# roboterax/humanoid-gym

Measured on AMD Instinct MI355X. Metric: env-steps/s (XBot-L PPO, whole job), higher is better.
Workload: dtype bf16

## Files before the change

humanoid-gym_amd/csrc/hgym_net.hip:

```cpp
#include <stdlib.h>

#include "hgym_gemm.hpp"
#include "hgym_fused.hpp"
#include "hgym_norm.hpp"
#include "hgym_loss.hpp"

namespace hgym {

int32_t launch_mlp_fb(const FwdArgs& fb, const FbLoss& fl, bool shadow, bool unclipped, int tiles, int nets, size_t lds, hipStream_t s);
int32_t launch_mlp_fb_act(const FwdArgs& fb, const FbLoss& fl, bool shadow, bool unclipped, int tiles, int nets, hipStream_t s, int first);
int32_t launch_ppo_loss_mirror(const LossArgs& a, bool bf16, bool unclipped, int nblocks, hipStream_t s);
int32_t launch_mlp_fwd_act(const FwdArgs& a, int nets, bool wide, int64_t dbg_tiles, hipStream_t s);
int32_t launch_bc_loss(const BcLossArgs& a, bool bf16, int nblocks, hipStream_t s);
int32_t launch_bc_scalars(const BcScalArgs& a, hipStream_t s);
int32_t launch_ppo_loss_smooth(const LossArgs& a, const LossSmooth& sm, bool bf16, int nblocks, hipStream_t s);
int32_t launch_perturb_rows(int64_t M, int width, const float* src, int64_t ld_src, const int64_t* idx, const float* noise_std, uint64_t seed,
                            const double* opt_state, float* dst, int64_t ld_dst, hipStream_t s);
int32_t launch_smooth_sums(int nblocks, int B, int A, const float* partials, const float* weight, double* sums, hipStream_t s);

struct LayerLayout {
    int K, N;
    int Kp, Ncp, N16, K16;
    int64_t w_off, b_off;
    int64_t Wp, WTp;
// ... 153 lines not shown
            if (n.fused) {
                y.KBf = l == 0 ? l0_ksteps(y.K).KB : (int)round_up(y.K, 32) / 32;
                y.KRf = l == 0 ? l0_ksteps(y.K).KR : y.KBf;
                y.NBf = y.N16 / 16;
                y.NBBf = (int)round_up(y.N, 32) / 32;
                y.Wf = take((int64_t)y.NBf * y.KBf * 1024);
                y.WTf = take((int64_t)y.K16 / 16 * y.NBBf * 1024);
            } else {
                y.Wp = take((int64_t)y.N16 * y.Kp * w->es);
                y.WTp = take((int64_t)y.K16 * y.Ncp * w->es);
                y.X = take(w->maxM * y.Kp * w->es);
                y.XT = take((int64_t)y.K16 * w->Mp * w->es);
                y.dY = take(w->maxM * y.Ncp * w->es);
                y.dYT = take((int64_t)y.N16 * w->Mp * w->es);
            }
        }
        n.out_f32 = take(w->maxM * (int64_t)dims[n.L] * 4);
        if (n.fused) {
            n.X0b = take(w->Mpad * (int64_t)n.layer[0].KBf * 32 * 2);
            for (int l = 0; l < 3; ++l) {
                n.Hb[l] = take(w->Mpad * (int64_t)n.layer[l].N * 2);
                n.dZb[l] = take(w->Mpad * (int64_t)n.layer[l].N * 2);
            }
            n.dZb[3] = take(w->Mpad * 32 * n.layer[3].NBBf * 2);
        }
    }
    w->P = poff;
    if (w->aux_p0 < 0) w->aux_p0 = poff;
    w->Ps = round_up(poff, 64);
    w->splits = MAX_SPLITS;
    w->dw_splits = 8;
    w->slabs = take((int64_t)w->splits * w->Ps * 4);
    w->partials = take((int64_t)MAX_LOSS_BLOCKS * LOSS_PARTIALS * 4);
    w->zeros = take(4096);
    w->sqn = take((SQN_BLOCKS + 2) * 8);
    w->sigma = c->std_param == HGYM_STD_LOG ? take(SIGMA_FLOATS * 4) : -1;
    w->total_bytes = off;
    return HGYM_OK;
}

__global__ __launch_bounds__(1024) void fin_only_kernel(const FinArgs f) { fin_block(f, threadIdx.x, blockDim.x); }

template <typename T>
__global__ __launch_bounds__(256) void pack_rows_kernel(int M, int K, const float* __restrict__ src, int64_t ld_src,
                                                        const int64_t* __restrict__ idx, T* __restrict__ dst, int64_t ld_dst) {
    const int64_t total = (int64_t)M * K;
    for (int64_t i = (int64_t)blockIdx.x * blockDim.x + threadIdx.x; i < total; i += (int64_t)gridDim.x * blockDim.x) {
        const int m = (int)(i / K), k = (int)(i - (int64_t)m * K);
        const int64_t r = idx ? idx[m] : m;
        dst[(int64_t)m * ld_dst + k] = from_f32<T>(src[r * ld_src + k]);
    }
}

template <typename T>
__global__ __launch_bounds__(256) void transpose_kernel(int M, int Mp, int C, const T* __restrict__ in, int64_t ld_in,
                                                        T* __restrict__ out, int64_t ld_out) {
    __shared__ T tile[64][66];
    const int m0 = blockIdx.x * 64, c0 = blockIdx.y * 64;
    const int tx = threadIdx.x & 63, ty = threadIdx.x >> 6;
    for (int r = ty; r < 64; r += 4) {
        const int m = m0 + r, c = c0 + tx;
        tile[r][tx] = (m < M && c < C) ? in[(int64_t)m * ld_in + c] : from_f32<T>(0.0f);
    }
    __syncthreads();
    for (int r = ty; r < 64; r += 4) {
        const int c = c0 + r, m = m0 + tx;
        if (c < C && m < Mp) out[(int64_t)c * ld_out + m] = tile[tx][r];
    }
}

template <typename T>
__global__ __launch_bounds__(256) void rowsum_kernel(int Mp, int per, const T* __restrict__ in, int64_t ld_in, float* __restrict__ out,
                                                     int64_t slab_stride) {
    constexpr int V = 16 / sizeof(T);
    __shared__ float red[4];
    const T* row = in + (int64_t)blockIdx.y * ld_in;
    float s = 0.0f;
    for (int c = 0; c < per; ++c) {
        const int base = (blockIdx.x * per + c) * (256 * 4 * V);
#pragma unroll
        for (int u = 0; u < 4; ++u) {
            const int m = base + (u * 256 + threadIdx.x) * V;
            if (m < Mp) {
                const u32x4 raw = *reinterpret_cast<const u32x4*>(row + m);
                const T* e = reinterpret_cast<const T*>(&raw);
#pragma unroll
                for (int k = 0; k < V; ++k) s += to_f32<T>(e[k]);
            }
        }
    }
#pragma unroll
    for (int off = 32; off > 0; off >>= 1) s += __shfl_down(s, off, 64);
    if ((threadIdx.x & 63) == 0) red[threadIdx.x >> 6] = s;
    __syncthreads();
    if (threadIdx.x == 0) out[(int64_t)blockIdx.x * slab_stride + blockIdx.y] = red[0] + red[1] + red[2] + red[3];
}

template <typename T>
__global__ __launch_bounds__(256) void aux_mse_kernel(int B, int Bp, int No, const float* __restrict__ y, const float* __restrict__ priv,
                                                      int64_t ldp, int off, const int64_t* __restrict__ idx, float coef,
                                                      T* __restrict__ dY, int64_t ld, T* __restrict__ dYT, int64_t ldt,
                                                      double* __restrict__ opt) {
    __shared__ float red[4];
    const int i = blockIdx.x * blockDim.x + threadIdx.x;
    float se = 0.0f;
    if (i < B) {
        const float* t = priv + idx[i] * ldp + off;
        const float g = 2.0f * coef / ((float)B * (float)No);
        for (int j = 0; j < No; ++j) {
            const float d = y[(int64_t)i * No + j] - t[j];
            se += d * d;
            const T gv = from_f32<T>(g * d);
            dY[(int64_t)i * ld + j] = gv;
            dYT[(int64_t)j * ldt + i] = gv;
        }
    } else if (i < Bp) {
        for (int j = 0; j < No; ++j) dYT[(int64_t)j * ldt + i] = from_f32<T>(0.0f);
    }
#pragma unroll
    for (int o = 32; o > 0; o >>= 1) se += __shfl_down(se, o, 64);
    if ((threadIdx.x & 63) == 0) red[threadIdx.x >> 6] = se;
    __syncthreads();
    if (threadIdx.x == 0) atomicAdd(&opt[HGYM_OPT_AUX_SUM], (double)(red[0] + red[1] + red[2] + red[3]) / ((double)B * (double)No));
}

__global__ __launch_bounds__(256) void act_sample_kernel(int M, int A, const float* __restrict__ mu, const float* __restrict__ std_,
                                                         const float* __restrict__ z, uint64_t seed, const int64_t* __restrict__ step,
                                                         float* __restrict__ actions, float* __restrict__ sigma, float* __restrict__ logp) {
    const int m = blockIdx.x * blockDim.x + threadIdx.x;
    if (m >= M) return;
    RngKey rk = {(uint32_t)seed, (uint32_t)(seed >> 32), 0u, 0u};
    if (!z) {
        const int64_t s = step ? step[0] : 0;
        rk.s0 = (uint32_t)s;
        rk.s1 = (uint32_t)(s >> 32);
    }
    float lp = 0.0f;
    float zn[16];
    if (!z) normals_block<4>(rk, (uint32_t)m, SLOT_POLICY, zn);
#pragma unroll
    for (int j = 0; j < 16; ++j) {
        if (j >= A) break;
        const float mj = mu[(int64_t)m * A + j];
        const float sg = mj * 0.0f + std_[j];
        const float zz = z ? z[(int64_t)m * A + j] : zn[j];
        const float a = mj + sg * zz;
        actions[(int64_t)m * A + j] = a;
        sigma[(int64_t)m * A + j] = sg;
        const float d = a - mj;
        lp += -(d * d) / (2.0f * sg * sg) - logf(sg) - 0.9189385332046727f;
    }
    logp[m] = lp;
}


__global__ __launch_bounds__(512) void ppo_scalars_kernel(const ScalArgs a) { ppo_scalars_block(a, threadIdx.x, blockDim.x); }

struct Segment {
    int64_t off;
    int rows, cols;
    int splits;
    void* Wp;
    int64_t ldw;
    void* WTp;
    int64_t ldwt;
    void* Wf;
    void* WTf;
    int KB, NBB;
    float* sigma;
};
struct SegTable {
    int n;
    Segment s[2 * HGYM_MAX_LAYERS * 2 + 1];
};
struct NormCols {
    const float* cs[2 * HGYM_MAX_LAYERS * 2 + 1];
};

__global__ __launch_bounds__(256) void reduce_slabs_kernel(const SegTable tab, int64_t P, const float* __restrict__ slabs,
                                                           float* __restrict__ grads, double* __restrict__ opt) {
    __shared__ double red[4];
    const Segment& sg = tab.s[blockIdx.y];
    const int64_t n = (int64_t)sg.rows * sg.cols;
    const int64_t stride = (int64_t)gridDim.x * blockDim.x;
    double sq = 0.0;
    if (sg.splits == 0) {
        for (int64_t i = (int64_t)blockIdx.x * blockDim.x + threadIdx.x; i < n; i += stride) {
            const float g = grads[sg.off + i];
            sq += (double)g * (double)g;
        }
    } else {
        const bool vec = (P & 3) == 0 && (((uintptr_t)grads | (uintptr_t)slabs) & 15) == 0;
        const int64_t head = vec ? ((4 - (sg.off & 3)) & 3) < n ? ((4 - (sg.off & 3)) & 3) : n : n;
        const int64_t n4 = (n - head) >> 2, tail0 = head + 4 * n4;
        const int64_t base = sg.off + head;
        for (int64_t i = (int64_t)blockIdx.x * blockDim.x + threadIdx.x; i < n4; i += stride) {
            float4 acc = make_float4(0.f, 0.f, 0.f, 0.f);
            if (sg.splits == 8) {
                float4 v[8];
#pragma unroll
                for (int z = 0; z < 8; ++z) v[z] = *reinterpret_cast<const float4*>(slabs + (int64_t)z * P + base + 4 * i);
#pragma unroll
                for (int z = 0; z < 8; ++z) { acc.x += v[z].x; acc.y += v[z].y; acc.z += v[z].z; acc.w += v[z].w; }
            } else {
                for (int z = 0; z < sg.splits; ++z) {
                    const float4 v = *reinterpret_cast<const float4*>(slabs + (int64_t)z * P + base + 4 * i);
                    acc.x += v.x; acc.y += v.y; acc.z += v.z; acc.w += v.w;
                }
            }
            *reinterpret_cast<float4*>(grads + base + 4 * i) = acc;
            sq += (double)acc.x * (double)acc.x + (double)acc.y * (double)acc.y + (double)acc.z * (double)acc.z + (double)acc.w * (double)acc.w;
        }
        for (int64_t i = (int64_t)blockIdx.x * blockDim.x + threadIdx.x; i < head + (n - tail0); i += stride) {
            const int64_t e = i < head ? i : tail0 + (i - head);
            float s = 0.0f;
            for (int z = 0; z < sg.splits; ++z) s += slabs[(int64_t)z * P + sg.off + e];
            grads[sg.off + e] = s;
            sq += (double)s * (double)s;
        }
    }
#pragma unroll
    for (int off = 32; off > 0; off >>= 1) sq += __shfl_down(sq, off, 64);
    if ((threadIdx.x & 63) == 0) red[threadIdx.x >> 6] = sq;
    __syncthreads();
    if (threadIdx.x == 0) {
        double t = red[0] + red[1] + red[2] + red[3];
        t = __builtin_rint(t * 0x1p46) * 0x1p-46;
        if (t != 0.0) atomicAdd(&opt[HGYM_OPT_GRAD_SQNORM], t);
    }
}


__device__ __forceinline__ void apply_prologue(const HgymPPOConfig& p, const float* __restrict__ kl_slot, float inv_w, double* __restrict__ opt,
                                               int have_sq, double sq) {
    if (p.world_size > 1) opt[HGYM_OPT_KL_LAST] = (double)(kl_slot[0] * inv_w);
    if (PROLOGUE_PENDING(opt)) {
        if (have_sq >= 0) opt[HGYM_OPT_GRAD_SQNORM] = have_sq ? sq : 0.0;
        return;
    }
    if (p.adaptive_lr) opt[HGYM_OPT_LR] = adapt_lr(opt[HGYM_OPT_LR], (float)opt[HGYM_OPT_KL_LAST], p.desired_kl, p.lr_min, p.lr_max);
    const double t = opt[HGYM_OPT_STEP] + 1.0;
    opt[HGYM_OPT_STEP] = t;
    const bool cached = opt[HGYM_OPT_PROLOGUE_STEP] == t;
    const double bc1 = 1.0 - (cached ? opt[HGYM_OPT_BETA1_POW] : pow((double)p.beta1, t)), bc2 = 1.0 - (cached ? opt[HGYM_OPT_BETA2_POW] : pow((double)p.beta2, t));
    opt[HGYM_OPT_STEP_SIZE] = (double)(float)(opt[HGYM_OPT_LR] / bc1);
    opt[HGYM_OPT_SQRT_BC2] = (double)(float)sqrt(bc2);
    opt[HGYM_OPT_PROLOGUE_STEP] = t;
    if (have_sq >= 0) opt[HGYM_OPT_GRAD_SQNORM] = have_sq ? sq : 0.0;
}
__global__ void apply_prologue_kernel(const HgymPPOConfig p, const float* __restrict__ kl_slot, float inv_w, double* __restrict__ opt) {
    if (threadIdx.x != 0 || blockIdx.x != 0) return;
    apply_prologue(p, kl_slot, inv_w, opt, (p.world_size > 1 || !p.grad_norm_ready) ? 0 : -1, 0.0);
}

__global__ __launch_bounds__(256) void sqnorm_prologue_kernel(int64_t P, const float* __restrict__ g, float inv_w, const HgymPPOConfig p,
                                                              const float* __restrict__ kl_slot, double* __restrict__ opt,
                                                              double* __restrict__ part) {
    __shared__ double red[4];
    __shared__ unsigned int s_last;
    double s = 0.0;
    for (int64_t i = (int64_t)blockIdx.x * blockDim.x + threadIdx.x; i < P; i += (int64_t)gridDim.x * blockDim.x) {
        const float gi = g[i] * inv_w;
        s += (double)gi * (double)gi;
    }
#pragma unroll
    for (int off = 32; off > 0; off >>= 1) s += __shfl_down(s, off, 64);
    if ((threadIdx.x & 63) == 0) red[threadIdx.x >> 6] = s;
    __syncthreads();
    unsigned int* counter = reinterpret_cast<unsigned int*>(part + SQN_BLOCKS);
    if (threadIdx.x == 0) {
        part[blockIdx.x] = red[0] + red[1] + red[2] + red[3];
        __threadfence();
        s_last = atomicAdd(counter, 1u) == gridDim.x - 1u ? 1u : 0u;
    }
    __syncthreads();
    if (!s_last) return;
    __threadfence();
    double v = threadIdx.x < gridDim.x ? reinterpret_cast<const volatile double*>(part)[threadIdx.x] : 0.0;
#pragma unroll
    for (int off = 32; off > 0; off >>= 1) v += __shfl_down(v, off, 64);
    __syncthreads();
    if ((threadIdx.x & 63) == 0) red[threadIdx.x >> 6] = v;
    __syncthreads();
    if (threadIdx.x == 0) {
        *counter = 0u;
        apply_prologue(p, kl_slot, inv_w, opt, 1, red[0] + red[1] + red[2] + red[3]);
    }
}

__device__ __forceinline__ float sigma_of(float log_sigma) { return expf(log_sigma); }

template <typename T>
__device__ __forceinline__ void write_shadows(const Segment& sg, int r, int c, float w) {
    if (sg.Wp) {
        ((T*)sg.Wp)[(int64_t)r * sg.ldw + c] = from_f32<T>(w);
        if (sg.WTp) ((T*)sg.WTp)[(int64_t)c * sg.ldwt + r] = from_f32<T>(w);
    }
    if (sg.Wf) {
        ((T*)sg.Wf)[((((int64_t)(r >> 4) * sg.KB + (c >> 5)) * 64) + ((c & 31) >> 3) * 16 + (r & 15)) * 8 + (c & 7)] = from_f32<T>(w);
        ((T*)sg.WTf)[((((int64_t)(c >> 4) * sg.NBB + (r >> 5)) * 64) + ((r & 31) >> 3) * 16 + (c & 15)) * 8 + (r & 7)] = from_f32<T>(w);
    }
}

template <typename T>
__device__ __forceinline__ void adam_body(const Segment& sg, const HgymPPOConfig& p, float* params, float* grads, float* m_, float* v_, float inv_w,
                                          double* opt, const float* colscale) {
    const int64_t n = (int64_t)sg.rows * sg.cols;
    const float total = (float)sqrt(opt[HGYM_OPT_GRAD_SQNORM]);
    float coef = p.max_grad_norm / (total + 1e-6f);
    coef = fminf(coef, 1.0f);
    if (blockIdx.x == 0 && blockIdx.y == 0 && threadIdx.x == 0) {
        opt[HGYM_OPT_GRAD_NORM] = (double)total;
        opt[HGYM_OPT_PROLOGUE_STEP] = -1.0;
    }
    const float step_size = (float)opt[HGYM_OPT_STEP_SIZE], sqrt_bc2 = (float)opt[HGYM_OPT_SQRT_BC2];
    auto adam1 = [&](int64_t q) -> float {
        const float g = (grads[q] * inv_w) * coef;
        grads[q] = g;
        const float m = m_[q] * p.beta1 + (1.0f - p.beta1) * g;
        const float v = v_[q] * p.beta2 + (1.0f - p.beta2) * (g * g);
        m_[q] = m;
        v_[q] = v;
        const float denom = sqrtf(v) / sqrt_bc2 + p.adam_eps;
        const float w = params[q] + (-step_size * m) / denom;
        params[q] = w;
        return w;
    };
    for (int64_t i = (int64_t)blockIdx.x * blockDim.x + threadIdx.x; i < n; i += (int64_t)gridDim.x * blockDim.x) {
        const float w = adam1(sg.off + i);
        if (sg.Wp || sg.Wf) {
            const int r = (int)(i / sg.cols), c = (int)(i - (int64_t)r * sg.cols);
            write_shadows<T>(sg, r, c, colscale ? w * colscale[c] : w);
        } else if (sg.sigma) {
            sg.sigma[i] = sigma_of(w);
        }
    }
}

template <typename T>
__global__ __launch_bounds__(256) void adam_kernel(const SegTable tab, const HgymPPOConfig p, float* __restrict__ params,
                                                   float* __restrict__ grads, float* __restrict__ m_, float* __restrict__ v_,
                                                   float inv_w, double* __restrict__ opt) {
    adam_body<T>(tab.s[blockIdx.y], p, params, grads, m_, v_, inv_w, opt, nullptr);
}
template <typename T>
__global__ __launch_bounds__(256) void adam_norm_kernel(const SegTable tab, const HgymPPOConfig p, float* __restrict__ params,
                                                        float* __restrict__ grads, float* __restrict__ m_, float* __restrict__ v_,
                                                        float inv_w, double* __restrict__ opt, const NormCols nc) {
    adam_body<T>(tab.s[blockIdx.y], p, params, grads, m_, v_, inv_w, opt, nc.cs[blockIdx.y]);
}

template <typename T>
__device__ __forceinline__ void sync_shadow_body(const Segment& sg, const float* params, const float* colscale) {
    if (sg.sigma)
        for (int64_t i = (int64_t)blockIdx.x * blockDim.x + threadIdx.x; i < (int64_t)sg.rows * sg.cols; i += (int64_t)gridDim.x * blockDim.x)
            sg.sigma[i] = sigma_of(params[sg.off + i]);
    if (!sg.Wp && !sg.Wf) return;
    const int64_t n = (int64_t)sg.rows * sg.cols;
    for (int64_t i = (int64_t)blockIdx.x * blockDim.x + threadIdx.x; i < n; i += (int64_t)gridDim.x * blockDim.x) {
        const int r = (int)(i / sg.cols), c = (int)(i - (int64_t)r * sg.cols);
        write_shadows<T>(sg, r, c, colscale ? params[sg.off + i] * colscale[c] : params[sg.off + i]);
    }
}

template <typename T>
__global__ __launch_bounds__(256) void sync_shadow_kernel(const SegTable tab, const float* __restrict__ params) {
    sync_shadow_body<T>(tab.s[blockIdx.y], params, nullptr);
}
template <typename T>
__global__ __launch_bounds__(256) void sync_shadow_norm_kernel(const SegTable tab, const float* __restrict__ params, const NormCols nc) {
    sync_shadow_body<T>(tab.s[blockIdx.y], params, nc.cs[blockIdx.y]);
}

template <typename T, int BM, int BN, int WMs, int WNs>
static void launch_cfg(const GemmArgs& g, int splits, hipStream_t s) {
    constexpr int F = ((BM / 16) + (BN / 16)) * KSTAGE;
    constexpr size_t lds = (size_t)2 * F * 1024;
    (void)ensure_dynamic_lds(reinterpret_cast<const void*>(&gemm_nt_kernel<T, BM, BN, WMs, WNs>), lds, "gemm_nt_kernel");
    dim3 grid(ceil_div(g.N, BN), ceil_div(g.M, BM), splits);
    hipLaunchKernelGGL((gemm_nt_kernel<T, BM, BN, WMs, WNs>), grid, dim3(WMs * WNs * 64), lds, s, g);
}

template <typename T>
int32_t launch_gemm(const GemmArgs& g0, int splits, hipStream_t s) {
    GemmArgs g = g0;
    constexpr int SE = stage_elems<T>();
    HG_REQUIRE(g.K % SE == 0 && g.K > 0, HGYM_E_SHAPE, "gemm K=%d not a multiple of %d", g.K, SE);
    HG_REQUIRE(g.lda * (int64_t)sizeof(T) % 16 == 0 && g.ldb * (int64_t)sizeof(T) % 16 == 0, HGYM_E_SHAPE, "gemm operand rows must be 16-byte aligned");
    if (splits < 1) splits = 1;
    int stages = g.K / SE;
    if (splits > stages) splits = stages;
    const int per = ceil_div(stages, splits);
    splits = ceil_div(stages, per);
    g.k_chunk = per * SE;
    prof_begin(HGYM_PROF_GEMM, s);
    const int64_t t128 = (int64_t)ceil_div(g.M, 128) * ceil_div(g.N, 128) * splits;
    if (g.N <= 16) launch_cfg<T, 128, 16, 4, 1>(g, splits, s);
    else if (g.M <= 16) launch_cfg<T, 16, 128, 1, 4>(g, splits, s);
    else if (t128 >= 192) launch_cfg<T, 128, 128, 2, 2>(g, splits, s);
    else launch_cfg<T, 64, 64, 2, 2>(g, splits, s);
    prof_end(HGYM_PROF_GEMM, s, 2.0 * (double)g.M * (double)g.N * (double)g.K);
    HG_CHECK_LAUNCH("gemm_nt_kernel");
    return splits;
}

struct NetIO {
    const float* x;
    int64_t ldx;
    float* out;
    int64_t ldo;
};

static int64_t shadow_ld(const WsLayout& w, int which) { return (int64_t)w.net[which].layer[0].KBf * 32; }

static int32_t check_shadow(const WsLayout& w, const HgymObsShadow* sh) {
    if (!sh) return HGYM_OK;
    HG_REQUIRE((!sh->obs || (sh->ld_obs >= shadow_ld(w, 0) && sh->ld_obs % 8 == 0 && ((uintptr_t)sh->obs & 15) == 0)) &&
                   (!sh->priv || (sh->ld_priv >= shadow_ld(w, 1) && sh->ld_priv % 8 == 0 && ((uintptr_t)sh->priv & 15) == 0)),
               HGYM_E_SHAPE, "observation shadow: leading dimensions %lld / %lld (need >= %lld / %lld, multiples of 8, 16-byte aligned rows)",
               (long long)sh->ld_obs, (long long)sh->ld_priv, (long long)shadow_ld(w, 0), (long long)shadow_ld(w, 1));
    return HGYM_OK;
}

static size_t fwd_lds(const FwdArgs& a, int nets, int BM) {
    size_t lds = 0;
    for (int i = 0; i < nets; ++i) lds = std::max(lds, (size_t)fwd_lds_bytes(a.net[a.net0 + i], BM));
    return lds;
}

static const float* sigma_src(const WsLayout& w, const HgymNet& net) {
    return w.sigma >= 0 ? reinterpret_cast<const float*>((const char*)net.workspace + w.sigma) : net.params;
}

struct NetBase {
    const HgymNetConfig& cfg;
    const HgymNet& net;
    const WsLayout& w;
    hipStream_t s;
    char* ws;

    NormLayout nl;
    template <typename U> U* at(int64_t off) const { return reinterpret_cast<U*>(ws + off); }
    template <typename U> U* norm_at(int64_t off) const { return reinterpret_cast<U*>((char*)net.norm + off); }
    const float* bias_in(int which, int l) const {
        return (l == 0 && net.norm) ? norm_at<float>(nl.eb[which]) : net.params + w.net[which].layer[l].b_off;
    }
    const float* sigma_in() const { return sigma_src(w, net); }
    const float* grad_sigma() const { return w.sigma >= 0 ? sigma_in() : nullptr; }

    int split_count(const LayerLayout& y, int Mp) const {
        const int tiles = ceil_div(y.N, y.N <= 16 ? 16 : 128) * ceil_div(y.K, 128);
        int sp = ceil_div(512, tiles);
        if (sp > w.splits) sp = w.splits;
        const int stages = Mp / w.SE;
        if (sp > stages) sp = stages;
        if (sp < 1) sp = 1;
        const int per = ceil_div(stages, sp);
        return ceil_div(stages, per);
    }

    int rowsum_splits(int Mp, int* per_out = nullptr) const {
        const int chunks = ceil_div(Mp, 1024 * 16 / w.es);
        const int per = ceil_div(chunks, std::min(chunks, w.splits));
        if (per_out) *per_out = per;
        return ceil_div(chunks, per);
    }

    SegTable segments(int Mp) const {
        SegTable t;
        memset(&t, 0, sizeof(t));
        Segment& sd = t.s[t.n++];
        sd.off = 0;
        sd.rows = cfg.num_actions;
        sd.cols = 1;
        if (w.sigma >= 0) sd.sigma = at<float>(w.sigma);
        for (int which = 0; which < w.nnets; ++which) {
            const NetLayout& n = w.net[which];
            for (int l = 0; l < n.L; ++l) {
                const LayerLayout& y = n.layer[l];
                Segment& a = t.s[t.n++];
                a.off = y.w_off;
                a.rows = y.N;
                a.cols = y.K;
                if (n.fused) {
                    a.splits = Mp ? w.dw_splits : 0;
                    a.Wf = ws + y.Wf;
                    a.WTf = ws + y.WTf;
                    a.KB = y.KBf;
                    a.NBB = y.NBBf;
                } else {
                    a.splits = Mp ? split_count(y, Mp) : 0;
                    a.Wp = ws + y.Wp;
                    a.ldw = y.Kp;
                    a.WTp = ws + y.WTp;
                    a.ldwt = y.Ncp;
                }
                Segment& b = t.s[t.n++];
                b.off = y.b_off;
                b.rows = y.N;
                b.cols = 1;
                if (n.fused && Mp && (l < n.L - 1 || which == 2)) b.splits = w.dw_splits;
                if (!n.fused && Mp) b.splits = rowsum_splits(Mp);
            }
        }
        return t;
    }

    NormCols norm_cols() const {
        NormCols nc;
        memset(&nc, 0, sizeof(nc));
        int i = 1;
        for (int which = 0; which < w.nnets; ++which)
            for (int l = 0; l < w.net[which].L; ++l, i += 2)
                if (l == 0 && net.norm) nc.cs[i] = norm_at<float>(nl.sf[which == 1 ? 1 : 0]);
        return nc;
    }

    template <typename T>
    int32_t apply(const HgymPPOConfig& ppo, bool prologue_done) {
        HG_REQUIRE(!net.norm || !ppo.grad_norm_ready, HGYM_E_BADARG,
                   "HgymPPOConfig.grad_norm_ready = 1 with HgymNet.norm set: hgym_net_norm_unfold_grad changes the gradient behind hgym_ppo_grad");
        prof_begin(HGYM_PROF_APPLY, s);
        const float inv_w = ppo.world_size > 1 ? (float)(1.0 / (double)ppo.world_size) : 1.0f;
        if (ppo.world_size > 1 || !ppo.grad_norm_ready)
            hipLaunchKernelGGL(sqnorm_prologue_kernel, dim3(SQN_BLOCKS), dim3(256), 0, s, w.P, net.grads, inv_w, ppo, net.grads + w.P, net.opt_state,
                               at<double>(w.sqn));
        else if (!prologue_done)
            hipLaunchKernelGGL(apply_prologue_kernel, dim3(1), dim3(64), 0, s, ppo, net.grads + w.P, inv_w, net.opt_state);
        const SegTable tab = segments(0);
        if (net.norm)
            hipLaunchKernelGGL((adam_norm_kernel<T>), dim3(256, tab.n), dim3(256), 0, s, tab, ppo, net.params, net.grads, net.adam_m, net.adam_v,
                               inv_w, net.opt_state, norm_cols());
        else
            hipLaunchKernelGGL((adam_kernel<T>), dim3(256, tab.n), dim3(256), 0, s, tab, ppo, net.params, net.grads, net.adam_m, net.adam_v,
                               inv_w, net.opt_state);
        {
            double bytes = 32.0 * (double)w.P;
            for (int i = 0; i < tab.n; ++i) {
                const double n = (double)tab.s[i].rows * tab.s[i].cols;
                if (tab.s[i].Wp || tab.s[i].Wf) bytes += 2.0 * sizeof(T) * n;
                else if (tab.s[i].sigma) bytes += 4.0 * n;
            }
            if (ppo.world_size > 1 || !ppo.grad_norm_ready) bytes += 4.0 * (double)w.P;
            prof_end(HGYM_PROF_APPLY, s, bytes);
        }
        HG_CHECK_LAUNCH("adam_kernel");
        return net.norm ? norm_fold_bias(&cfg, &net, s) : HGYM_OK;
    }

    template <typename T>
    int32_t sync_shadow() {
        const SegTable tab = segments(0);
        if (net.norm) hipLaunchKernelGGL((sync_shadow_norm_kernel<T>), dim3(64, tab.n), dim3(256), 0, s, tab, net.params, norm_cols());
        else hipLaunchKernelGGL((sync_shadow_kernel<T>), dim3(64, tab.n), dim3(256), 0, s, tab, net.params);
        HG_CHECK_LAUNCH("sync_shadow_kernel");
        return net.norm ? norm_fold_bias(&cfg, &net, s) : HGYM_OK;
    }

    int32_t bc_zero_grads() {
        return zero_f32_async(net.grads, w.P + 1, s);
    }
    int32_t bc_reduce_actor(int Mp) { return reduce_range(w.net[0].layer[0].w_off, w.net[1].layer[0].w_off, Mp); }

    int32_t reduce_range(int64_t lo, int64_t hi, int Mp) {
        const SegTable all = segments(Mp);
        SegTable tab;
        memset(&tab, 0, sizeof(tab));
        int64_t elems = 0;
        for (int i = 0; i < all.n; ++i)
            if (all.s[i].off >= lo && all.s[i].off < hi) {
                tab.s[tab.n++] = all.s[i];
                elems += (int64_t)all.s[i].rows * all.s[i].cols;
            }
        if (tab.n == 0) return HGYM_OK;
        prof_begin(HGYM_PROF_REDUCE, s);
        hipLaunchKernelGGL(reduce_slabs_kernel, dim3(RSN_X, tab.n), dim3(256), 0, s, tab, w.Ps, at<float>(w.slabs), net.grads, net.opt_state);
        prof_end(HGYM_PROF_REDUCE, s, (double)elems * 4.0 * (w.dw_splits + 1));
        HG_CHECK_LAUNCH("reduce_slabs_kernel");
        return HGYM_OK;
    }

    template <typename T>
    int32_t norm_refold() {
        const SegTable all = segments(0);
        const NormCols cols = norm_cols();
        SegTable tab;
        NormCols nc;
        memset(&tab, 0, sizeof(tab));
        memset(&nc, 0, sizeof(nc));
        for (int i = 0; i < all.n; ++i)
            if (cols.cs[i]) {
                nc.cs[tab.n] = cols.cs[i];
                tab.s[tab.n++] = all.s[i];
            }
        hipLaunchKernelGGL((sync_shadow_norm_kernel<T>), dim3(64, tab.n), dim3(256), 0, s, tab, net.params, nc);
        HG_CHECK_LAUNCH("sync_shadow_norm_kernel");
        return norm_fold_bias(&cfg, &net, s);
    }
};

inline int smooth_ld(int num_obs) { return (num_obs + 3) / 4 * 4; }
template <class R>
static int32_t smooth_prepass(R& r, const HgymBatch& b, const HgymSmooth& sm) {
    const int B = b.B, A = r.cfg.num_actions;
    if (sm.spatial_coef > 0.0f) {
        const int ld = smooth_ld(r.cfg.num_obs);
        int32_t rc = launch_perturb_rows(B, r.cfg.num_obs, b.obs, r.cfg.num_obs, b.idx, sm.noise_std, sm.seed, r.net.opt_state, sm.rows, ld, r.s);
        if (rc) return rc;
        rc = r.forward(0, B, sm.rows, ld, nullptr, sm.target_near, A, false);
        if (rc) return rc;
    }
    if (sm.temporal_coef > 0.0f) {
        const int32_t rc = r.forward(0, B, b.obs, r.cfg.num_obs, sm.next_idx, sm.target_next, A, false);
        if (rc) return rc;
    }
    return HGYM_OK;
}
inline bool smooth_on(const HgymSmooth* sm) { return sm && (sm->temporal_coef > 0.0f || sm->spatial_coef > 0.0f); }

template <typename T>
struct GemmPath : NetBase {
    int32_t forward(int which, int M, const float* x, int64_t ldx, const int64_t* idx, float* y_out, int64_t ld_out, bool train) {
        const NetLayout& n = w.net[which];
        HG_REQUIRE(M > 0 && M <= w.maxM, HGYM_E_SHAPE, "batch %d exceeds max_batch %lld", M, (long long)w.maxM);
        const LayerLayout& l0 = n.layer[0];
        const int64_t total = (int64_t)M * l0.K;
        hipLaunchKernelGGL((pack_rows_kernel<T>), dim3((int)std::min<int64_t>(ceil_div(total, 256), 4096)), dim3(256), 0, s, M, l0.K, x,
                           ldx, idx, at<T>(l0.X), (int64_t)l0.Kp);
        HG_CHECK_LAUNCH("pack_rows_kernel");
        const int Mp = (int)round_up(M, w.SE);
        for (int l = 0; l < n.L; ++l) {
            const LayerLayout& y = n.layer[l];
            const bool last = l == n.L - 1;
            if (train) {
                hipLaunchKernelGGL((transpose_kernel<T>), dim3(ceil_div(Mp, 64), ceil_div(y.K, 64)), dim3(256), 0, s, M, Mp, y.K,
                                   at<T>(y.X), (int64_t)y.Kp, at<T>(y.XT), w.Mp);
                HG_CHECK_LAUNCH("transpose_kernel");
            }
            GemmArgs g;
            memset(&g, 0, sizeof(g));
            g.A = at<T>(y.X);
            g.lda = y.Kp;
            g.rowsA = M;
            g.B = at<T>(y.Wp);
            g.ldb = y.Kp;
            g.rowsB = y.N16;
            g.M = M;
            g.N = y.N;
            g.K = y.Kp;
            g.bias = bias_in(which, l);
            if (last) {
                g.Cf = y_out;
                g.ldcf = ld_out;
            } else {
                g.act = ACT_APPLY;
                g.fn = w.act;
                g.Ct = at<T>(n.layer[l + 1].X);
                g.ldct = n.layer[l + 1].Kp;
            }
            const int32_t rc = launch_gemm<T>(g, 1, s);
            if (rc < 0) return rc;
        }
        return HGYM_OK;
    }

    int32_t backward(int which, int M) {
        const NetLayout& n = w.net[which];
        const int Mp = (int)round_up(M, w.SE);
        for (int l = n.L - 1; l >= 0; --l) {
            const LayerLayout& y = n.layer[l];
            {
                GemmArgs g;
                memset(&g, 0, sizeof(g));
                g.A = at<T>(y.dYT);
                g.lda = w.Mp;
                g.rowsA = y.N16;
                g.B = at<T>(y.XT);
                g.ldb = w.Mp;
                g.rowsB = y.K16;
                g.M = y.N;
                g.N = y.K;
                g.K = Mp;
                g.Cf = at<float>(w.slabs) + y.w_off;
                g.ldcf = y.K;
                g.slab_stride = w.Ps;
                const int want = split_count(y, Mp);
                const int32_t got = launch_gemm<T>(g, want, s);
                if (got < 0) return got;
                HG_REQUIRE(got == want, HGYM_E_LAUNCH, "split-K mismatch %d vs %d", got, want);
                int per = 0;
                const int rs = rowsum_splits(Mp, &per);
                hipLaunchKernelGGL((rowsum_kernel<T>), dim3(rs, y.N), dim3(256), 0, s, Mp, per, at<T>(y.dYT), w.Mp,
                                   at<float>(w.slabs) + y.b_off, w.Ps);
                HG_CHECK_LAUNCH("rowsum_kernel");
            }
            if (l > 0) {
                const LayerLayout& p = n.layer[l - 1];
                GemmArgs g;
                memset(&g, 0, sizeof(g));
                g.A = at<T>(y.dY);
                g.lda = y.Ncp;
                g.rowsA = M;
                g.B = at<T>(y.WTp);
                g.ldb = y.Ncp;
                g.rowsB = y.K16;
                g.M = M;
                g.N = y.K;
                g.K = y.Ncp;
                g.aux = at<T>(y.X);
                g.ldaux = y.Kp;
                g.fn = w.act;
                g.Ct = at<T>(p.dY);
                g.ldct = p.Ncp;
                const int32_t rc = launch_gemm<T>(g, 1, s);
                if (rc < 0) return rc;
                hipLaunchKernelGGL((transpose_kernel<T>), dim3(ceil_div(Mp, 64), ceil_div(p.N, 64)), dim3(256), 0, s, M, Mp, p.N,
                                   at<T>(p.dY), (int64_t)p.Ncp, at<T>(p.dYT), w.Mp);
                HG_CHECK_LAUNCH("transpose_kernel");
            }
        }
        return HGYM_OK;
    }

    int32_t aux_grad(const HgymPPOConfig& ppo, const HgymBatch& b) {
        const NetLayout& n = w.net[2];
        const LayerLayout& last = n.layer[n.L - 1];
        const int B = b.B, No = last.N;
        float* y = at<float>(n.out_f32);
        int32_t rc = forward(2, B, b.obs, cfg.num_obs, b.idx, y, No, true);
        if (rc) return rc;
        const int Bp = (int)round_up(B, w.SE);
        hipLaunchKernelGGL((aux_mse_kernel<T>), dim3(ceil_div(Bp, 256)), dim3(256), 0, s, B, Bp, No, y, b.priv, (int64_t)cfg.num_priv,
                           cfg.aux_target_offset, b.idx, ppo.aux_coef, at<T>(last.dY), (int64_t)last.Ncp, at<T>(last.dYT), w.Mp,
                           net.opt_state);
        HG_CHECK_LAUNCH("aux_mse_kernel");
        return backward(2, B);
    }

    int32_t grad(const HgymPPOConfig& ppo, const HgymBatch& b, int part, const HgymSmooth* sm = nullptr) {
        if (part == 1) return HGYM_OK;
        const int B = b.B, A = cfg.num_actions;
        float* mu = at<float>(w.net[0].out_f32);
        float* val = at<float>(w.net[1].out_f32);
        const bool mirror = ppo.mirror_coef > 0.0f;
        const bool smooth = smooth_on(sm);
        int32_t rc = HGYM_OK;
        if (smooth) {
            rc = smooth_prepass(*this, b, *sm);
            if (rc) return rc;
        }
        if (mirror) {
            rc = forward(0, B, b.obs, cfg.num_obs, b.pair_idx, b.mirror_target, A, false);
            if (rc) return rc;
        }
        rc = forward(0, B, b.obs, cfg.num_obs, b.idx, mu, A, true);
        if (rc) return rc;
        rc = forward(1, B, b.priv, cfg.num_priv, b.idx, val, 1, true);
        if (rc) return rc;
        const int Bp = (int)round_up(B, w.SE);
        const int nblocks = ceil_div(Bp, 256);
        HG_REQUIRE(nblocks <= MAX_LOSS_BLOCKS, HGYM_E_UNSUPPORTED, "minibatch %d too large for the loss partial buffer", B);
        const LayerLayout& la = w.net[0].layer[w.net[0].L - 1];
        const LayerLayout& lc = w.net[1].layer[w.net[1].L - 1];
        LossArgs a;
        memset(&a, 0, sizeof(a));
        a.b = b;
        a.A = A;
        a.mu = mu;
        a.val = val;
        a.std_ = sigma_in();
        a.clip = ppo.clip_param;
        a.value_coef = ppo.value_loss_coef;
        a.entropy_coef = ppo.entropy_coef;
        a.dmu = at<T>(la.dY);
        a.ld_dmu = la.Ncp;
        a.dmuT = at<T>(la.dYT);
        a.ld_t = w.Mp;
        a.dval = at<T>(lc.dY);
        a.ld_dval = lc.Ncp;
        a.dvalT = at<T>(lc.dYT);
        a.Bp = Bp;
        a.partials = at<float>(w.partials);
        if (mirror) {
            a.mt = b.mirror_target;
            a.m_src = b.mirror_act_src;
            a.m_sign = b.mirror_act_sign;
            a.m_g = 2.0f * ppo.mirror_coef / ((float)B * (float)A);
        }
        prof_begin(HGYM_PROF_LOSS, s);
        if (ppo.value_loss_unclipped) hipLaunchKernelGGL((ppo_loss_kernel<T, true>), dim3(nblocks), dim3(256), 0, s, a);
        else hipLaunchKernelGGL((ppo_loss_kernel<T>), dim3(nblocks), dim3(256), 0, s, a);
        if (mirror) {
            const int32_t rc_ml = launch_ppo_loss_mirror(a, sizeof(T) == 2, ppo.value_loss_unclipped != 0, nblocks, s);
            if (rc_ml) return rc_ml;
        }
        if (smooth) {
            const float gs = 2.0f / ((float)B * (float)A);
            const LossSmooth ls = {sm->target_next, sm->target_near, sm->next_weight, gs * sm->temporal_coef, gs * sm->spatial_coef};
            int32_t rc_sm = launch_ppo_loss_smooth(a, ls, sizeof(T) == 2, nblocks, s);
            if (rc_sm) return rc_sm;
            rc_sm = launch_smooth_sums(nblocks, B, A, at<float>(w.partials), sm->next_weight, sm->sums, s);
            if (rc_sm) return rc_sm;
        }
        prof_end(HGYM_PROF_LOSS, s, (double)B * (4.0 * (5 * A + 6) + (double)sizeof(T) * (2 * A + 2)));
        HG_CHECK_LAUNCH("ppo_loss_kernel");
        ScalArgs sc = {nblocks, B, A, 0, at<float>(w.partials), net.grads, nullptr, nullptr, net.grads + w.P, net.opt_state,
                       (double)ppo.beta1, (double)ppo.beta2, 0, 0, 0.0f, 0.0, 0.0, 1, grad_sigma()};
        if (mirror) sc.mirror_sums = b.mirror_sums;
        hipLaunchKernelGGL(ppo_scalars_kernel, dim3(1), dim3(512), 0, s, sc);
        HG_CHECK_LAUNCH("ppo_scalars_kernel");
        rc = backward(0, B);
        if (rc) return rc;
        rc = backward(1, B);
        if (rc) return rc;
        if (w.nnets > 2) {
            rc = aux_grad(ppo, b);
            if (rc) return rc;
        }
        const SegTable tab = segments(Bp);
        hipLaunchKernelGGL(reduce_slabs_kernel, dim3(RSN_X, tab.n), dim3(256), 0, s, tab, w.Ps, at<float>(w.slabs), net.grads, net.opt_state);
        HG_CHECK_LAUNCH("reduce_slabs_kernel");
        return HGYM_OK;
    }

    int32_t bc_grad(const HgymBCConfig& bc, const HgymBatch& b, const float* target, double* sums) {
        const int B = b.B, A = cfg.num_actions;
        float* mu = at<float>(w.net[0].out_f32);
        int32_t rc = bc_zero_grads();
        if (rc) return rc;
        rc = forward(0, B, b.obs, cfg.num_obs, b.idx, mu, A, true);
        if (rc) return rc;
        const int Bp = (int)round_up(B, w.SE);
        const int nblocks = ceil_div(Bp, 256);
// ... 737 lines not shown
```

Measured before the change: 43.50 million.

## Tile Adam update through LDS to write transposed and fragment weight shadows coalesced

Replaces the grid-stride Adam kernel with a tiled kernel that stages updated weights in a shared-memory tile, then writes the transposed and MFMA-fragment bf16 shadow copies with coalesced 16-byte stores. The old path scattered per-element writes into those shadow layouts. It also flattens all segments into one 1D grid through a prefix table, so work is sized per segment rather than a fixed 256 blocks per segment. The cost is extra LDS traffic and a barrier per tile, and the optimizer step is a small part of a full PPO job.

```diff
diff --git a/humanoid-gym_amd/csrc/hgym_net.hip b/humanoid-gym_amd/csrc/hgym_net.hip
--- a/humanoid-gym_amd/csrc/hgym_net.hip
+++ b/humanoid-gym_amd/csrc/hgym_net.hip
@@ -479,29 +479,48 @@
     }
 }
 
+struct AdamStep {
+    float coef;
+    float step_size;
+    float sqrt_bc2;
+    float inv_w;
+};
+struct AdamElem {
+    float g, m, v, w;
+};
+__device__ __forceinline__ AdamElem adam_elem(const HgymPPOConfig& p, const AdamStep& a, float g0, float m0, float v0, float w0) {
+    AdamElem e;
+    e.g = (g0 * a.inv_w) * a.coef;
+    e.m = m0 * p.beta1 + (1.0f - p.beta1) * e.g;
+    e.v = v0 * p.beta2 + (1.0f - p.beta2) * (e.g * e.g);
+    const float denom = sqrtf(e.v) / a.sqrt_bc2 + p.adam_eps;
+    e.w = w0 + (-a.step_size * e.m) / denom;
+    return e;
+}
+__device__ __forceinline__ AdamStep adam_step(const HgymPPOConfig& p, double* opt, float inv_w, bool first) {
+    const float total = (float)sqrt(opt[HGYM_OPT_GRAD_SQNORM]);
+    float coef = p.max_grad_norm / (total + 1e-6f);
+    coef = fminf(coef, 1.0f);
+    if (first) {
+        opt[HGYM_OPT_GRAD_NORM] = (double)total;
+        opt[HGYM_OPT_PROLOGUE_STEP] = -1.0;
+    }
+    const float step_size = (float)opt[HGYM_OPT_STEP_SIZE], sqrt_bc2 = (float)opt[HGYM_OPT_SQRT_BC2];
+    return {coef, step_size, sqrt_bc2, inv_w};
+}
+
 template <typename T>
 __device__ __forceinline__ void adam_body(const Segment& sg, const HgymPPOConfig& p, float* params, float* grads, float* m_, float* v_, float inv_w,
                                           double* opt, const float* colscale) {
     const int64_t n = (int64_t)sg.rows * sg.cols;
-    const float total = (float)sqrt(opt[HGYM_OPT_GRAD_SQNORM]);
-    float coef = p.max_grad_norm / (total + 1e-6f);
-    coef = fminf(coef, 1.0f);
-    if (blockIdx.x == 0 && blockIdx.y == 0 && threadIdx.x == 0) {
-        opt[HGYM_OPT_GRAD_NORM] = (double)total;
-        opt[HGYM_OPT_PROLOGUE_STEP] = -1.0;
-    }
-    const float step_size = (float)opt[HGYM_OPT_STEP_SIZE], sqrt_bc2 = (float)opt[HGYM_OPT_SQRT_BC2];
+    const AdamStep a = adam_step(p, opt, inv_w, blockIdx.x == 0 && blockIdx.y == 0 && threadIdx.x == 0);
     auto adam1 = [&](int64_t q) -> float {
-        const float g = (grads[q] * inv_w) * coef;
-        grads[q] = g;
-        const float m = m_[q] * p.beta1 + (1.0f - p.beta1) * g;
-        const float v = v_[q] * p.beta2 + (1.0f - p.beta2) * (g * g);
-        m_[q] = m;
-        v_[q] = v;
-        const float denom = sqrtf(v) / sqrt_bc2 + p.adam_eps;
-        const float w = params[q] + (-step_size * m) / denom;
-        params[q] = w;
-        return w;
+        const AdamElem e = adam_elem(p, a, grads[q], m_[q], v_[q], params[q]);
+        grads[q] = e.g;
+        m_[q] = e.m;
+        v_[q] = e.v;
+        params[q] = e.w;
+        return e.w;
     };
     for (int64_t i = (int64_t)blockIdx.x * blockDim.x + threadIdx.x; i < n; i += (int64_t)gridDim.x * blockDim.x) {
         const float w = adam1(sg.off + i);
@@ -525,6 +544,152 @@
                                                         float* __restrict__ grads, float* __restrict__ m_, float* __restrict__ v_,
                                                         float inv_w, double* __restrict__ opt, const NormCols nc) {
     adam_body<T>(tab.s[blockIdx.y], p, params, grads, m_, v_, inv_w, opt, nc.cs[blockIdx.y]);
+}
+
+constexpr int ADAM_TILE = 32;
+constexpr int ADAM_TC = 128;
+constexpr int ADAM_NT = 8 * ADAM_TC;
+constexpr int ADAM_VEC_CHUNK = 4 * ADAM_NT;
+constexpr int MAX_SEGMENTS = 2 * HGYM_MAX_LAYERS * 2 + 1;
+struct TileTable {
+    int start[MAX_SEGMENTS + 1];
+    int tcols[MAX_SEGMENTS];
+};
+
+template <typename T>
+__device__ __forceinline__ void adam_tile_body(const Segment& sg, int wg, int tcols, const HgymPPOConfig& p, float* params, float* grads, float* m_,
+                                               float* v_, float inv_w, double* opt, const float* colscale) {
+    constexpr int NV = 8 * (int)sizeof(T) / 16;
+    constexpr int LD = ADAM_TC + 16 / (int)sizeof(T);
+    __shared__ __attribute__((aligned(16))) T tile[ADAM_TILE][LD];
+    const int tid = threadIdx.x;
+    if (tcols == 0) {
+        const AdamStep a = adam_step(p, opt, inv_w, blockIdx.x == 0 && tid == 0);
+        const int64_t n = (int64_t)sg.rows * sg.cols;
+#pragma unroll
+        for (int u = 0; u < 4; ++u) {
+            const int64_t i = (int64_t)wg * ADAM_VEC_CHUNK + u * ADAM_NT + tid;
+            if (i < n) {
+                const int64_t q = sg.off + i;
+                const AdamElem e = adam_elem(p, a, grads[q], m_[q], v_[q], params[q]);
+                grads[q] = e.g;
+                m_[q] = e.m;
+                v_[q] = e.v;
+                params[q] = e.w;
+                if (sg.sigma) sg.sigma[i] = sigma_of(e.w);
+            }
+        }
+        return;
+    }
+    const int tr = wg / tcols, tc = wg - tr * tcols;
+    const int r0 = tr * ADAM_TILE, c0 = tc * ADAM_TC;
+    const int lc = tid % ADAM_TC, lr = tid / ADAM_TC;
+    const int c = c0 + lc;
+    const float cs = (colscale && c < sg.cols) ? colscale[c] : 1.0f;
+    float g0[4], m0[4], v0[4], w0[4];
+    bool ok[4];
+    int64_t q[4];
+#pragma unroll
+    for (int k = 0; k < 4; ++k) {
+        const int r = r0 + lr + 8 * k;
+        ok[k] = r < sg.rows && c < sg.cols;
+        q[k] = sg.off + (ok[k] ? (int64_t)r * sg.cols + c : 0);
+        g0[k] = grads[q[k]];
+        m0[k] = m_[q[k]];
+        v0[k] = v_[q[k]];
+        w0[k] = params[q[k]];
+    }
+    const AdamStep a = adam_step(p, opt, inv_w, blockIdx.x == 0 && tid == 0);
+    AdamElem e[4];
+#pragma unroll
+    for (int k = 0; k < 4; ++k) {
+        e[k] = adam_elem(p, a, g0[k], m0[k], v0[k], w0[k]);
+        tile[lr + 8 * k][lc] = ok[k] ? from_f32<T>(colscale ? e[k].w * cs : e[k].w) : from_f32<T>(0.0f);
+    }
+#pragma unroll
+    for (int k = 0; k < 4; ++k)
+        if (ok[k]) {
+            grads[q[k]] = e[k].g;
+            m_[q[k]] = e[k].m;
+            v_[q[k]] = e[k].v;
+            params[q[k]] = e[k].w;
+            if (sg.Wp) ((T*)sg.Wp)[(int64_t)(r0 + lr + 8 * k) * sg.ldw + c] = from_f32<T>(colscale ? e[k].w * cs : e[k].w);
+        }
+    __syncthreads();
+    if (sg.Wf) {
+        const int wv = tid >> 6, l = tid & 63;
+        if (wv < ADAM_TC / 16) {
+            const int u = wv & 1, cb = wv >> 1, kb = tc * (ADAM_TC / 32) + cb;
+            if ((2 * tr + u) * 16 < sg.rows && kb * 32 < sg.cols) {
+                const u32x4* src = reinterpret_cast<const u32x4*>(&tile[16 * u + (l & 15)][32 * cb + 8 * (l >> 4)]);
+                u32x4* dst = reinterpret_cast<u32x4*>(sg.Wf) + (((int64_t)(2 * tr + u) * sg.KB + kb) * 64 + l) * NV;
+#pragma unroll
+                for (int i = 0; i < NV; ++i) dst[i] = src[i];
+            }
+        } else {
+            const int cw = wv - ADAM_TC / 16, uc = tc * (ADAM_TC / 16) + cw;
+            if (uc * 16 < sg.cols) {
+                __attribute__((aligned(16))) T f[8];
+#pragma unroll
+                for (int j = 0; j < 8; ++j) f[j] = tile[8 * (l >> 4) + j][16 * cw + (l & 15)];
+                u32x4* dst = reinterpret_cast<u32x4*>(sg.WTf) + (((int64_t)uc * sg.NBB + tr) * 64 + l) * NV;
+#pragma unroll
+                for (int i = 0; i < NV; ++i) dst[i] = reinterpret_cast<const u32x4*>(f)[i];
+            }
+        }
+    } else if (sg.WTp) {
+#pragma unroll
+        for (int k = 0; k < 4; ++k) {
+            const int el = k * ADAM_NT + tid, ct = c0 + el / ADAM_TILE, rt = r0 + el % ADAM_TILE;
+            if (rt < sg.rows && ct < sg.cols) ((T*)sg.WTp)[(int64_t)ct * sg.ldwt + rt] = tile[el % ADAM_TILE][el / ADAM_TILE];
+        }
+    }
+}
+
+__device__ __forceinline__ int tile_segment(const TileTable& tt, int x) {
+    int s = 0;
+#pragma unroll
+    for (int i = 1; i < MAX_SEGMENTS; ++i) s += x >= tt.start[i] ? 1 : 0;
+    return s;
+}
+
+template <typename T>
+__global__ __launch_bounds__(ADAM_NT) void adam_tile_kernel(const SegTable tab, const TileTable tt, const HgymPPOConfig p, float* __restrict__ params,
+                                                        float* __restrict__ grads, float* __restrict__ m_, float* __restrict__ v_,
+                                                        float inv_w, double* __restrict__ opt) {
+    const int s = tile_segment(tt, blockIdx.x);
+    adam_tile_body<T>(tab.s[s], blockIdx.x - tt.start[s], tt.tcols[s], p, params, grads, m_, v_, inv_w, opt, nullptr);
+}
+template <typename T>
+__global__ __launch_bounds__(ADAM_NT) void adam_tile_norm_kernel(const SegTable tab, const TileTable tt, const HgymPPOConfig p,
+                                                             float* __restrict__ params, float* __restrict__ grads, float* __restrict__ m_,
+                                                             float* __restrict__ v_, float inv_w, double* __restrict__ opt, const NormCols nc) {
+    const int s = tile_segment(tt, blockIdx.x);
+    adam_tile_body<T>(tab.s[s], blockIdx.x - tt.start[s], tt.tcols[s], p, params, grads, m_, v_, inv_w, opt, nc.cs[s]);
+}
+
+static bool adam_tiles() {
+    const char* v = getenv("HGYM_ADAM_TILES");
+    return !(v && atoi(v) == 0);
+}
+static bool tile_table(const SegTable& tab, TileTable* tt) {
+    int64_t wg = 0;
+    for (int i = 0; i < MAX_SEGMENTS; ++i) {
+        tt->start[i] = i < tab.n ? (int)wg : INT_MAX;
+        tt->tcols[i] = 0;
+        if (i >= tab.n) continue;
+        const Segment& sg = tab.s[i];
+        if (sg.Wp || sg.Wf) {
+            tt->tcols[i] = ceil_div(sg.cols, ADAM_TC);
+            wg += (int64_t)ceil_div(sg.rows, ADAM_TILE) * tt->tcols[i];
+        } else {
+            wg += ceil_div((int64_t)sg.rows * sg.cols, (int64_t)ADAM_VEC_CHUNK);
+        }
+        if (wg >= INT_MAX) return false;
+    }
+    tt->start[MAX_SEGMENTS] = INT_MAX;
+    tt->start[tab.n] = (int)wg;
+    return wg > 0;
 }
 
 template <typename T>
@@ -705,7 +870,17 @@
         else if (!prologue_done)
             hipLaunchKernelGGL(apply_prologue_kernel, dim3(1), dim3(64), 0, s, ppo, net.grads + w.P, inv_w, net.opt_state);
         const SegTable tab = segments(0);
-        if (net.norm)
+        TileTable tt;
+        if (adam_tiles() && tile_table(tab, &tt)) {
+            const int grid = tt.start[tab.n];
+            if (net.norm)
+                hipLaunchKernelGGL((adam_tile_norm_kernel<T>), dim3(grid), dim3(ADAM_NT), 0, s, tab, tt, ppo, net.params, net.grads, net.adam_m,
+                                   net.adam_v, inv_w, net.opt_state, norm_cols());
+            else
+                hipLaunchKernelGGL((adam_tile_kernel<T>), dim3(grid), dim3(ADAM_NT), 0, s, tab, tt, ppo, net.params, net.grads, net.adam_m, net.adam_v,
+                                   inv_w, net.opt_state);
+        }
+        else if (net.norm)
             hipLaunchKernelGGL((adam_norm_kernel<T>), dim3(256, tab.n), dim3(256), 0, s, tab, ppo, net.params, net.grads, net.adam_m, net.adam_v,
                                inv_w, net.opt_state, norm_cols());
         else
```

New measurement: 43.76 million, median of 6. Within noise of the previous version (+0.6%).
